# VIS4ROB-lab/ccm_slam

Measured on AMD Instinct MI355X. Metric: global-BA LM iterations/s (4-agent merged map), higher is better.
Workload: dtype f64; 1 GPU; gba_c4: global BA (MapFusionGBA numerics), 2000 KFs / 150000 landmarks / 954782 observations, Huber sqrt(5.99), landmark-sharded x1

## Files before the change

ccm_slam_amd/csrc/ba.hip:

```cpp
#include "common.h"
#include "test_internal.h"
#include "ba_types.h"
#include "lane_xor.h"
#include "ba_math.h"
#include <algorithm>
#include <chrono>
#include <cmath>
#include <cstring>
#include <limits>
#include <numeric>

int ccm_allreduce_f64(ccm_ctx* ctx, double* d_buf, size_t n);
int ccm_allreduce_max_f64(ccm_ctx* ctx, double* d_buf, size_t n);

namespace {


inline double now_ms() {
  return std::chrono::duration<double, std::milli>(std::chrono::steady_clock::now().time_since_epoch()).count();
}

__device__ __forceinline__ double wave_sum(double v) { return lanex::wave_sum(v); }

__device__ __forceinline__ double block_sum(double v, double* lds ) {
// ... 2634 lines not shown
    if (d.chunk_off) hipLaunchKernelGGL(ba_backsub_chi2_e, dim3(d.n_chunk), dim3(kTPB), 0, ctx->stream, d, ba->cur, 0.0, 1);
    else hipLaunchKernelGGL(ba_backsub_chi2, dim3(d.n_wg_pt), dim3(kTPB), 0, ctx->stream, d, ba->cur, 0.0, 1);
  }
  hipMemsetAsync(d.part_cam, 0, sizeof(double) * d.n_wg_cam, ctx->stream);
  const bool poll = ba->nranks == 1 && poll_enabled();
  const unsigned long long ticket = ++ba->rb_ticket;
  hipLaunchKernelGGL(ba_reduce_scalars, dim3(1), dim3(kTPB), 0, ctx->stream, d, ba->stop_local(), 0, 0, poll ? ba->h_rb : (double*)nullptr, ticket);
  RC(ba_allreduce_sum(ba, d.scal, 4));
  double s[6];
  if (poll) { RC(read_scalars_polled(ba, s, nullptr, ticket)); } else { RC(read_scalars(ba, s)); }
  *chi = s[0];
  ba->stop_any = s[2] > 0.0;
  return CCM_OK;
}

int build_system(ccm_ba* ba, double lambda_next = -1.0) {
  ccm_ctx* ctx = ba->ctx;
  BaDev& d = ba->d;
  ba->dinv_done_lambda = -1.0;
  if (d.Lloc) {
    ccm_prof_scope ps(ctx, CCM_K_BA_LINEARIZE);
    if (d.chunk_off) {
      hipLaunchKernelGGL(ba_linearize_pts_e, dim3(d.n_chunk), dim3(kTPB), 0, ctx->stream, d, ba->cur, lambda_next);
      if (lambda_next >= 0.0) ba->dinv_done_lambda = lambda_next;
    } else hipLaunchKernelGGL(ba_linearize_pts, dim3(d.n_wg_pt), dim3(kTPB), 0, ctx->stream, d, ba->cur);
  }
  if (d.Cp) {
    ccm_prof_scope ps(ctx, CCM_K_BA_CAM);
    hipLaunchKernelGGL(ba_linearize_cams, dim3(d.n_wg_wave4), dim3(kTPB), 0, ctx->stream, d, ba->cur);
  }
  CCM_HIP_CHECK(ctx, hipGetLastError());
  return CCM_OK;
}

int max_diag(ccm_ba* ba, double* out) {
  ccm_ctx* ctx = ba->ctx;
  BaDev& d = ba->d;
  const double* hpp = d.Hpp;
  if (ba->nranks > 1 && d.Cp) {
    CCM_HIP_CHECK(ctx, hipMemcpyAsync(ba->d_hpp_full, d.Hpp, 36 * (size_t)d.Cp * sizeof(double), hipMemcpyDeviceToDevice, ctx->stream));
    RC(ba_allreduce_sum(ba, ba->d_hpp_full, 36 * (size_t)d.Cp));
    hpp = ba->d_hpp_full;
  }
  const int nb = std::max(1, std::min(d.n_wg_pt, 512));
  hipLaunchKernelGGL(ba_maxdiag, dim3(nb), dim3(kTPB), 0, ctx->stream, d, hpp, d.part_pt, nb, 0);
  hipLaunchKernelGGL(ba_maxdiag, dim3(1), dim3(kTPB), 0, ctx->stream, d, hpp, d.part_pt, nb, 1);
  RC(ba_allreduce_max(ba, d.scal + 4, 1));
  double s[6];
  RC(read_scalars(ba, s));
  *out = s[4];
  return CCM_OK;
}

__global__ void ba_f64_to_f32(const double* __restrict__ in, float* __restrict__ out, size_t n) {
  const size_t i = (size_t)blockIdx.x * blockDim.x + threadIdx.x;
  if (i < n) out[i] = (float)in[i];
}

int coarse_build(ccm_ba* ba, double lambda) {
  ccm_ctx* ctx = ba->ctx;
  BaDev& d = ba->d;
  ccm_prof_scope ps(ctx, CCM_K_BA_COARSE);
  const int Nc = ba->coarse_Nc, na = ba->coarse_na, nn = na + 1;
  hipLaunchKernelGGL(ba_coarse_P, dim3(ccm_div_up(d.Cp, kTPB)), dim3(kTPB), 0, ctx->stream, d, ba->cur, ba->d_cP);
  hipLaunchKernelGGL(ba_coarse_assemble, dim3(ba->coarse_ncb), dim3(kCoarseTPB), 0, ctx->stream, d, (const double*)ba->d_cP,
                     (const int*)ba->d_cb_off, (const int*)ba->d_cb_ent, ba->coarse_ncb, (const int*)ba->d_blk_i, (const int*)ba->d_blk_j, lambda, ba->d_cstage);
  hipLaunchKernelGGL(ba_coarse_sum, dim3(ccm_div_up((int64_t)Nc * Nc, kTPB)), dim3(kTPB), 0, ctx->stream, (const double*)ba->d_cstage, (const unsigned*)ba->d_cb_key,
                     ba->coarse_ncb, na, nn, ba->d_cA, Nc);
  CCM_HIP_CHECK(ctx, hipGetLastError());
  RC(ccm_dense_chol_inverse_dev(ctx, ba->d_cA, Nc, ba->d_cLinv, ba->d_cX, ba->d_cAinv, ba->d_cinfo));
  if (ba->d_cAinv32) {
    const size_t n = (size_t)Nc * Nc;
    hipLaunchKernelGGL(ba_f64_to_f32, dim3((unsigned)ccm_div_up((int64_t)n, kTPB)), dim3(kTPB), 0, ctx->stream, (const double*)ba->d_cAinv, ba->d_cAinv32, n);
    CCM_HIP_CHECK(ctx, hipGetLastError());
  }
  return CCM_OK;
}

int coarse_prepare(ccm_ba* ba, double lambda) {
  const double win = 16.0;
  const double win_up_env = 0.0;
  const double win_up = win_up_env > 0 ? win_up_env : (ba->pers_grid ? 64.0 : win);
  const bool need = !ba->coarse_reuse || !ba->coarse_valid || ba->coarse_stale_bad || lambda > win_up * ba->coarse_lambda_built || lambda < ba->coarse_lambda_built / win;
  ba->coarse_fresh = need;
  if (!need) return CCM_OK;
  RC(coarse_build(ba, lambda));
  ba->coarse_valid = true; ba->coarse_stale_bad = false; ba->coarse_lambda_built = lambda;
  return CCM_OK;
}

int lm_trial(ccm_ba* ba, double lambda, const ccm_ba_options& opt, double* temp_chi, double* scale, bool* ok, int* pcg_iters) {
  ccm_ctx* ctx = ba->ctx;
  BaDev& d = ba->d;
  const int cur = ba->cur;
  if (!ba->pers_grid && ba->pers_grid_built && ba->pers_cooldown > 0 && --ba->pers_cooldown == 0) ba->pers_grid = ba->pers_grid_built;
  if (d.Lloc && ba->dinv_done_lambda != lambda) {
    ccm_prof_scope ps(ctx, CCM_K_BA_DINV);
    hipLaunchKernelGGL(ba_dinv, dim3(d.n_wg_pt), dim3(kTPB), 0, ctx->stream, d, lambda);
  }
  ba->dinv_done_lambda = -1.0;
  *ok = true;
  *pcg_iters = 0;
  bool small_path = false, pers_trial = false, pers_launch_failed = false, cams_updated = false;
  int small_flags[4] = {0, 0, 0, 0};
  if (d.Cp) {
    RC(launch_schur(ba));
    RC(ba_allreduce_sum(ba, ba->d_red, ba->red_count));
    const double tol_default = 1e-8;
    const double tol = opt.pcg_rel_tol > 0 ? opt.pcg_rel_tol : tol_default;
    const int max_it = opt.pcg_max_iters > 0 ? opt.pcg_max_iters : 1000;
    int flags[4] = {0, 0, 0, 0};
    const bool dense2_on = true;
    if (ba->d_cholreg_L) {
      CCM_LDS_ATTR(ctx, CCM_LDS_BA_CHOLREG, ba_solve_cholreg, cholreg_lds_bytes());
      if (!ba->cholreg_table_built) {
        hipLaunchKernelGGL(ba_cholreg_table, dim3(1), dim3(kCRTPB), 0, ctx->stream, d, ba->d_cholreg_tab);
        ba->cholreg_table_built = true;
      }
      {
        ccm_prof_scope ps(ctx, CCM_K_BA_PCG_PERSIST);
        hipLaunchKernelGGL(ba_solve_cholreg, dim3(1), dim3(kCRTPB), cholreg_lds_bytes(), ctx->stream, d, lambda, ba->d_cholreg_L, (const int*)ba->d_cholreg_tab,
                           ccm_dbg("cholreg") ? (long long*)ba->d_cholreg_dbg : (long long*)nullptr, cur, ba->rank == 0 ? 1 : 0);
      }
      small_path = true;
      cams_updated = true;
    } else if (d.Cp > kSmallMaxCp && d.Cp <= kDense2MaxCp && ba->d_dense_T && ba->d_pers_coff && dense2_on) {
      CCM_LDS_ATTR(ctx, CCM_LDS_BA_DENSE2, ba_solve_dense2, dense2_lds_bytes());
      {
// ... 537 lines not shown
```

ccm_slam_amd/csrc/common.h:

```cpp
#pragma once
#include <hip/hip_runtime.h>
#if defined(__HIP_DEVICE_COMPILE__) && !defined(__gfx950__)
#error "libccm_hip.so is written for gfx950 (MI355X) only: build with --offload-arch=gfx950"
#endif
#include <stdint.h>
#include <map>
#include <cstring>
#include <string>
#include <vector>
#include <mutex>
#include "../../include/ccm_hip.h"

struct ccm_prof_slot {
  std::vector<std::pair<hipEvent_t, hipEvent_t>> pending;
  int64_t launches = 0;
  double total_ms = 0.0;
};

struct ccm_ctx {
  int device = 0;
  hipStream_t stream = nullptr;
  std::string err;
  int prof_class = -2;
  ccm_prof_slot prof[CCM_K_COUNT];
// ... 12 lines not shown
int ccm_set_error(ccm_ctx* ctx, int code, const std::string& msg);
bool ccm_dbg(const char* topic);

struct ccm_coresident_scope {
  ccm_ctx* ctx; bool chained = false;
  explicit ccm_coresident_scope(ccm_ctx* c);
  ~ccm_coresident_scope();
  ccm_coresident_scope(const ccm_coresident_scope&) = delete;
  ccm_coresident_scope& operator=(const ccm_coresident_scope&) = delete;
};
void ccm_coresident_note_abort(ccm_ctx* ctx);

#define CCM_HIP_CHECK(ctx, expr)                                                        \
  do {                                                                                  \
    hipError_t _e = (expr);                                                             \
    if (_e != hipSuccess)                                                               \
      return ccm_set_error((ctx), CCM_E_HIP,                                            \
                           std::string(#expr) + ": " + hipGetErrorString(_e) + " (" +   \
                               __FILE__ + ":" + std::to_string(__LINE__) + ")");        \
  } while (0)

enum { CCM_LDS_BA_ROW = 0, CCM_LDS_BA_ROW2 = 8, CCM_LDS_BA_SMALL, CCM_LDS_BA_TILES, CCM_LDS_PG_PRECOND, CCM_LDS_POSEOPT, CCM_LDS_SIM3OPT, CCM_LDS_BA_DENSE2, CCM_LDS_ORB_OCT, CCM_LDS_ORB_OCT2, CCM_LDS_BA_ROW3, CCM_LDS_BA_ROW4, CCM_LDS_POSEOPT1, CCM_LDS_BA_CHOLREG };
#define CCM_LDS_ATTR(ctx, bit, func, bytes)                                                                              \
  do {                                                                                                                   \
    if (!((ctx)->lds_attr_done & (1u << (bit)))) {                                                                       \
      CCM_HIP_CHECK((ctx), hipFuncSetAttribute((const void*)(func), hipFuncAttributeMaxDynamicSharedMemorySize, (int)(bytes))); \
      (ctx)->lds_attr_done |= 1u << (bit);                                                                               \
    }                                                                                                                    \
  } while (0)

struct ccm_prof_scope {
  ccm_ctx* ctx; int cls; hipStream_t st = nullptr; hipEvent_t e0 = nullptr, e1 = nullptr; bool on = false;
  ccm_prof_scope(ccm_ctx* c, int k, hipStream_t launch_stream = nullptr);
  ~ccm_prof_scope();
};

int ccm_scratch(ccm_ctx* ctx, size_t bytes, void** out);
int ccm_io_scratch(ccm_ctx* ctx, size_t bytes, void** out);
int ccm_pin_scratch(ccm_ctx* ctx, size_t bytes, void** out);
int ccm_pool_get(ccm_ctx* ctx, size_t bytes, void** out, size_t* actual);
void ccm_pool_put(ccm_ctx* ctx, void* p, size_t actual);
struct ccm_tile_plan {
  int T = 0;
  std::vector<int> h_col_off;
  std::vector<int> h_upd_off;
  std::vector<int> h_row_off;
  const int* d_col_rows = nullptr;
  const int* d_upd_pairs = nullptr;
  const int* d_row_cols = nullptr;
};
void ccm_tile_plan_symbolic(int T, const std::vector<char>& nz, ccm_tile_plan* plan, std::vector<int>* col_rows, std::vector<int>* upd_pairs,
                            std::vector<int>* row_cols);
int ccm_dense_chol_solve_dev(ccm_ctx* ctx, double* d_A, int N, double* d_b, double* d_linv, int* d_info, const ccm_tile_plan* plan = nullptr);
int ccm_dense_chol_inverse_dev(ccm_ctx* ctx, double* d_A, int N, double* d_linv, double* d_X, double* d_Ainv, int* d_info);
struct ccm_tsc {
  int T = 0, n_tiles = 0, n_levels = 0;
  std::vector<int> tid;
  std::vector<int> lvl_col_off, lvl_gt_off, lvl_pt_off;
  int *d_tid = nullptr, *d_cols = nullptr, *d_gt = nullptr, *d_gk_off = nullptr, *d_gk = nullptr, *d_pt = nullptr;
  int *d_rc_off = nullptr, *d_rc = nullptr, *d_cr_off = nullptr, *d_cr = nullptr;
  double *d_tiles = nullptr, *d_linv = nullptr;
  int* d_info = nullptr;
  std::vector<std::pair<void*, size_t>> blocks;
  ccm_ctx* owner = nullptr;
  ccm_tsc() = default;
  ccm_tsc(const ccm_tsc&) = delete;
  ccm_tsc& operator=(const ccm_tsc&) = delete;
  ~ccm_tsc();
};
int ccm_tsc_create(ccm_ctx* ctx, int T, const std::vector<char>& nz, ccm_tsc* out);
void ccm_tsc_destroy(ccm_ctx* ctx, ccm_tsc* p);
int ccm_tsc_clear(ccm_ctx* ctx, ccm_tsc* p);
int ccm_tsc_solve(ccm_ctx* ctx, ccm_tsc* p, double* d_b);
static inline size_t ccm_align256(size_t n) { return (n + 255) & ~(size_t)255; }

static inline int ccm_div_up(int64_t a, int64_t b) { return (int)((a + b - 1) / b); }
```

ccm_slam_amd/csrc/dense_chol.hip:

```cpp
#include "common.h"
#include "test_internal.h"
#include <cstdlib>
#include <cstring>
#include <vector>

namespace {

constexpr int NB = 64;
constexpr int LD = NB + 1;
constexpr int kTPB = 256;
typedef double v4d __attribute__((ext_vector_type(4)));

__device__ __forceinline__ void tile_abt(const double* As, const double* Bs, v4d acc[4], int wave, int lane) {
  const int i = lane & 15, kq = lane >> 4;
#pragma unroll 4
  for (int kk = 0; kk < NB / 4; kk++) {
    const int k = 4 * kk + kq;
    const double a = As[(16 * wave + i) * LD + k];
#pragma unroll
    for (int s = 0; s < 4; s++) {
      const double b = Bs[(16 * s + i) * LD + k];
      acc[s] = __builtin_amdgcn_mfma_f64_16x16x4f64(a, b, acc[s], 0, 0, 0);
    }
  }
}

__device__ __forceinline__ void load_tile(double* dst, const double* src, int ld_src) {
  double v[NB * NB / kTPB];
#pragma unroll
  for (int q = 0; q < NB * NB / kTPB; q++) { const int e = threadIdx.x + q * kTPB; v[q] = src[(size_t)(e / NB) * ld_src + e % NB]; }
#pragma unroll
  for (int q = 0; q < NB * NB / kTPB; q++) { const int e = threadIdx.x + q * kTPB; dst[(e / NB) * LD + e % NB] = v[q]; }
}

__device__ __forceinline__ double bcast64(double v, int lane) {
  const long long b = __double_as_longlong(v);
  const int lo = __builtin_amdgcn_readlane((int)(b & 0xffffffffll), lane), hi = __builtin_amdgcn_readlane((int)(b >> 32), lane);
  return __longlong_as_double(((long long)hi << 32) | (unsigned int)lo);
}
__device__ __forceinline__ void chol_diag_body(double* Ajj, size_t N, int j, double* Lg, int* info) {
  constexpr int LR = NB + 2;
  __shared__ __attribute__((aligned(16))) double L[NB * LR];
  __shared__ double rdiag[NB];
  const int lane = threadIdx.x & 63;
  const int wv = __builtin_amdgcn_readfirstlane(threadIdx.x >> 6);
  {
    double tmp[NB / 2];
#pragma unroll
    for (int r = 0; r < NB / 2; r++) tmp[r] = Ajj[(size_t)(wv * (NB / 2) + r) * N + lane];
#pragma unroll
    for (int r = 0; r < NB / 2; r++) L[(wv * (NB / 2) + r) * LR + lane] = tmp[r];
  }
  __syncthreads();
  int bad_col = 0;
  double row[NB], cur[NB], nxt[NB];
  double x[NB];
  if (wv == 0) {
#pragma unroll
    for (int k = 0; k < NB; k++) { row[k] = L[lane * LR + k]; cur[k] = 0.0; nxt[k] = 0.0; }
  }
  __syncthreads();
#pragma unroll
  for (int c = 0; c <= NB; c++) {
    if (wv == 0) {
      if (c < NB) {
        double acc[4] = {row[c], 0.0, 0.0, 0.0};
#pragma unroll
        for (int k = 0; k < c; k++) acc[k & 3] = __builtin_fma(-row[k], cur[k], acc[k & 3]);
        if (c + 1 < NB) {
#pragma unroll
          for (int k = 0; k < c; k++) nxt[k] = L[(c + 1) * LR + k];
        }
        const double sv = (acc[0] + acc[1]) + (acc[2] + acc[3]);
        double dd = bcast64(sv, c);
        if (!(dd > 0.0)) { if (!bad_col) bad_col = c + 1; dd = 1.0; }
        const double inv = rsqrt(dd), l = dd * inv;
        row[c] = (lane == c) ? l : sv * inv;
        L[lane * LR + c] = row[c];
        if (lane == c) rdiag[c] = inv;
        if (c + 1 < NB) nxt[c] = bcast64(row[c], c + 1);
#pragma unroll
        for (int k = 0; k <= c; k++) cur[k] = nxt[k];
      }
    } else if (c >= 1) {
      const int r = c - 1;
      const double* Lrow = L + r * LR;
      double acc[4] = {(r == lane) ? 1.0 : 0.0, 0.0, 0.0, 0.0};
#pragma unroll
      for (int k = 0; k < r; k++) acc[k & 3] = __builtin_fma(-Lrow[k], x[k], acc[k & 3]);
      x[r] = ((acc[0] + acc[1]) + (acc[2] + acc[3])) * rdiag[r];
      Lg[r * NB + lane] = x[r];
    }
    __syncthreads();
  }
  if (wv == 0) {
    if (bad_col && lane == 0 && *info == 0) *info = j * NB + bad_col;
#pragma unroll
    for (int r = 0; r < NB; r++) Ajj[(size_t)r * N + lane] = (lane <= r) ? L[r * LR + lane] : 0.0;
  }
}
__device__ __forceinline__ void chol_diag_body_blk(double* Ajj, size_t N, int j, double* Lg, int* info) {
  constexpr int LR = NB + 2, KB = 16;
  __shared__ __attribute__((aligned(16))) double L[NB * LR];
  __shared__ double rdiag[NB];
  const int lane = threadIdx.x & 63;
  const int wv = __builtin_amdgcn_readfirstlane(threadIdx.x >> 6);
  {
    double tmp[NB / 2];
#pragma unroll
    for (int r = 0; r < NB / 2; r++) tmp[r] = Ajj[(size_t)(wv * (NB / 2) + r) * N + lane];
#pragma unroll
    for (int r = 0; r < NB / 2; r++) L[(wv * (NB / 2) + r) * LR + lane] = tmp[r];
  }
  __syncthreads();
  constexpr int kBlocks = NB / KB;
  static_assert(NB % KB == 0 && kBlocks >= 1, "both waves must run the same whole number of 16-column blocks");
  if (wv == 0) {
    int bad_col = 0;
#pragma unroll
    for (int b = 0; b < kBlocks; b++) {
      const int c0 = KB * b;
      double row[KB];
#pragma unroll
      for (int c = 0; c < KB; c += 2) { const double2 v = *reinterpret_cast<const double2*>(&L[lane * LR + c0 + c]); row[c] = v.x; row[c + 1] = v.y; }
#pragma unroll 2
      for (int k = 0; k < c0; k += 2) {
        const double2 a2 = *reinterpret_cast<const double2*>(&L[lane * LR + k]);
#pragma unroll
        for (int c = 0; c < KB; c++) {
          const double2 l2 = *reinterpret_cast<const double2*>(&L[(c0 + c) * LR + k]);
          row[c] = __builtin_fma(-a2.y, l2.y, __builtin_fma(-a2.x, l2.x, row[c]));
        }
      }
#pragma unroll
      for (int c = 0; c < KB; c++) {
        double s0 = row[c], s1 = 0.0;
#pragma unroll
        for (int k = 0; k < c; k++) {
          const double m = bcast64(row[k], c0 + c);
          if (k & 1) s1 = __builtin_fma(-row[k], m, s1); else s0 = __builtin_fma(-row[k], m, s0);
        }
        const double sv = s0 + s1;
        double dd = bcast64(sv, c0 + c);
        if (!(dd > 0.0)) { if (!bad_col) bad_col = c0 + c + 1; dd = 1.0; }
        const double inv = rsqrt(dd);
        row[c] = (lane == c0 + c) ? dd * inv : sv * inv;
        if (lane == c0 + c) rdiag[c0 + c] = inv;
      }
#pragma unroll
      for (int c = 0; c < KB; c += 2) { double2 v; v.x = row[c]; v.y = row[c + 1]; *reinterpret_cast<double2*>(&L[lane * LR + c0 + c]) = v; }
      __syncthreads();
    }
    if (bad_col && lane == 0 && *info == 0) *info = j * NB + bad_col;
#pragma unroll
    for (int r = 0; r < NB; r++) Ajj[(size_t)r * N + lane] = (lane <= r) ? L[r * LR + lane] : 0.0;
  } else {
    double x[NB];
#pragma unroll
    for (int b = 0; b < kBlocks; b++) {
      __syncthreads();
#pragma unroll
      for (int rr = 0; rr < KB; rr++) {
        const int r = KB * b + rr;
        const double* Lrow = L + r * LR;
        double acc[4] = {(r == lane) ? 1.0 : 0.0, 0.0, 0.0, 0.0};
#pragma unroll
        for (int k = 0; k < r; k++) acc[k & 3] = __builtin_fma(-Lrow[k], x[k], acc[k & 3]);
        x[r] = ((acc[0] + acc[1]) + (acc[2] + acc[3])) * rdiag[r];
        Lg[r * NB + lane] = x[r];
        asm volatile("" ::: "memory");
// ... 134 lines not shown
  __shared__ double v[NB];
  const int t = threadIdx.x;
  const double* Li = Linv_all + (size_t)j * NB * NB;
  v[t] = b[(size_t)j * NB + t];
  __syncthreads();
  double s = 0;
  if (!transpose) { for (int k = 0; k <= t; k++) s += Li[t * NB + k] * v[k]; }
  else { for (int k = t; k < NB; k++) s += Li[k * NB + t] * v[k]; }
  b[(size_t)j * NB + t] = s;
}
__global__ __launch_bounds__(NB) void chol_solve_update(const double* A, int N, double* b, int j, int transpose, const int* list ) {
  __shared__ double v[NB];
  const int t = threadIdx.x;
  v[t] = b[(size_t)j * NB + t];
  __syncthreads();
  double s = 0;
  if (!transpose) {
    const int i = list ? list[blockIdx.x] : j + 1 + blockIdx.x;
    const double* Lij = A + ((size_t)i * NB + t) * N + (size_t)j * NB;
    for (int k = 0; k < NB; k++) s += Lij[k] * v[k];
    b[(size_t)i * NB + t] -= s;
  } else {
    const int k = list ? list[blockIdx.x] : blockIdx.x;
    const double* Ljk = A + ((size_t)j * NB) * N + (size_t)k * NB + t;
    for (int r = 0; r < NB; r++) s += Ljk[(size_t)r * N] * v[r];
    b[(size_t)k * NB + t] -= s;
  }
}

__device__ __forceinline__ void load_tile_t(double* dst, const double* src, int ld_src) {
  double v[NB * NB / kTPB];
#pragma unroll
  for (int q = 0; q < NB * NB / kTPB; q++) { const int e = threadIdx.x + q * kTPB; v[q] = src[(size_t)(e / NB) * ld_src + e % NB]; }
#pragma unroll
  for (int q = 0; q < NB * NB / kTPB; q++) { const int e = threadIdx.x + q * kTPB; dst[(e % NB) * LD + e / NB] = v[q]; }
}

__device__ __forceinline__ void tile_abt16(const double* As, const double* Bs, v4d& acc, int wave, int lane) {
  const int i = lane & 15, kq = lane >> 4;
#pragma unroll 4
  for (int kk = 0; kk < NB / 4; kk++) {
    const int k = 4 * kk + kq;
    acc = __builtin_amdgcn_mfma_f64_16x16x4f64(As[(16 * wave + i) * LD + k], Bs[i * LD + k], acc, 0, 0, 0);
  }
}
__device__ __forceinline__ void load_strip_t(double* dst, const double* src, int ld_src) {
  double v[NB * 16 / kTPB];
#pragma unroll
  for (int q = 0; q < NB * 16 / kTPB; q++) { const int e = threadIdx.x + q * kTPB; v[q] = src[(size_t)(e / 16) * ld_src + e % 16]; }
#pragma unroll
  for (int q = 0; q < NB * 16 / kTPB; q++) { const int e = threadIdx.x + q * kTPB; dst[(e % 16) * LD + e / 16] = v[q]; }
}

__global__ __launch_bounds__(kTPB) void chol_tri_diag(int N, const double* Linv_all, double* X) {
  const int j = blockIdx.x;
  for (int e = threadIdx.x; e < NB * NB; e += kTPB) X[((size_t)j * NB + e / NB) * N + (size_t)j * NB + e % NB] = Linv_all[(size_t)j * NB * NB + e];
}
__global__ __launch_bounds__(kTPB) void chol_tri_step(const double* A, int N, const double* Linv_all, double* X, int k) {
  __shared__ double As[NB * LD], Bs[16 * LD];
  const int nj = k + 1;
  const int i = k + 1 + (int)blockIdx.x / nj, j = (int)blockIdx.x % nj, c0 = 16 * blockIdx.y;
  const int wave = threadIdx.x >> 6, lane = threadIdx.x & 63;
  const int i16 = lane & 15, kq = lane >> 4;
  double* Xij = X + ((size_t)i * NB) * N + (size_t)j * NB + c0;
  v4d acc = {0, 0, 0, 0};
  if (j != k) {
#pragma unroll
    for (int r = 0; r < 4; r++) acc[r] = Xij[(size_t)(16 * wave + kq + 4 * r) * N + i16];
  }
  load_tile(As, A + ((size_t)i * NB) * N + (size_t)k * NB, N);
  load_strip_t(Bs, X + ((size_t)k * NB) * N + (size_t)j * NB + c0, N);
  __syncthreads();
  tile_abt16(As, Bs, acc, wave, lane);
  __syncthreads();
  if (i == k + 1) {
#pragma unroll
    for (int r = 0; r < 4; r++) Bs[i16 * LD + 16 * wave + kq + 4 * r] = acc[r];
    load_tile(As, Linv_all + (size_t)i * NB * NB, NB);
    __syncthreads();
    v4d out = {0, 0, 0, 0};
    tile_abt16(As, Bs, out, wave, lane);
#pragma unroll
    for (int r = 0; r < 4; r++) Xij[(size_t)(16 * wave + kq + 4 * r) * N + i16] = -out[r];
  } else {
#pragma unroll
    for (int r = 0; r < 4; r++) Xij[(size_t)(16 * wave + kq + 4 * r) * N + i16] = acc[r];
  }
}

__global__ __launch_bounds__(kTPB) void chol_xtx(const double* X, int N, double* Ainv) {
  __shared__ double As[NB * LD], Bs[16 * LD];
  const int T = N / NB;
  const int pi = blockIdx.x, c0 = 16 * blockIdx.y;
  int p = (int)((sqrtf(8.0f * (float)pi + 1.0f) - 1.0f) * 0.5f);
  while (p * (p + 1) / 2 > pi) p--;
  while ((p + 1) * (p + 2) / 2 <= pi) p++;
  const int q = pi - p * (p + 1) / 2;
  const int wave = threadIdx.x >> 6, lane = threadIdx.x & 63;
  const int i16 = lane & 15, kq = lane >> 4;
  v4d acc = {0, 0, 0, 0};
  for (int k = p; k < T; k++) {
    load_tile_t(As, X + ((size_t)k * NB) * N + (size_t)p * NB, N);
    load_strip_t(Bs, X + ((size_t)k * NB) * N + (size_t)q * NB + c0, N);
    __syncthreads();
    tile_abt16(As, Bs, acc, wave, lane);
    __syncthreads();
  }
#pragma unroll
  for (int r = 0; r < 4; r++) {
    const int row = 16 * wave + kq + 4 * r, col = c0 + i16;
    Ainv[((size_t)p * NB + row) * N + (size_t)q * NB + col] = acc[r];
    if (p != q) Ainv[((size_t)q * NB + col) * N + (size_t)p * NB + row] = acc[r];
  }
}

}

int ccm_dense_chol_solve_dev(ccm_ctx* ctx, double* d_A, int N, double* d_b, double* d_linv, int* d_info, const ccm_tile_plan* plan) {
  if (N % NB) return ccm_set_error(ctx, CCM_E_ARG, "dense cholesky: N must be a multiple of 64");
  const int T = N / NB;
  if (plan && (plan->T != T || T >= 32768)) return ccm_set_error(ctx, CCM_E_ARG, "dense cholesky: tile plan does not match");
  CCM_HIP_CHECK(ctx, hipMemsetAsync(d_info, 0, sizeof(int), ctx->stream));
  for (int j = 0; j < T; j++) {
    if (diag_blocked()) hipLaunchKernelGGL(chol_diag_wave_blk, dim3(1), dim3(128), 0, ctx->stream, d_A, N, j, d_linv, d_info);
    else hipLaunchKernelGGL(chol_diag_wave, dim3(1), dim3(128), 0, ctx->stream, d_A, N, j, d_linv, d_info);
    if (plan) {
      const int nr = plan->h_col_off[j + 1] - plan->h_col_off[j], np = plan->h_upd_off[j + 1] - plan->h_upd_off[j];
      if (nr) hipLaunchKernelGGL(chol_panel, dim3(nr), dim3(kTPB), 0, ctx->stream, d_A, N, j, (const double*)d_linv, plan->d_col_rows + plan->h_col_off[j]);
      if (np) hipLaunchKernelGGL(chol_update, dim3(np), dim3(kTPB), 0, ctx->stream, d_A, N, j, plan->d_upd_pairs + plan->h_upd_off[j]);
      continue;
    }
    const int rem = T - j - 1;
    if (rem > 0) {
      hipLaunchKernelGGL(chol_panel, dim3(rem), dim3(kTPB), 0, ctx->stream, d_A, N, j, (const double*)d_linv, (const int*)nullptr);
      hipLaunchKernelGGL(chol_update, dim3(rem * (rem + 1) / 2), dim3(kTPB), 0, ctx->stream, d_A, N, j, (const int*)nullptr);
    }
  }
  for (int j = 0; j < T; j++) {
    hipLaunchKernelGGL(chol_solve_diag, dim3(1), dim3(NB), 0, ctx->stream, d_b, j, (const double*)d_linv, 0);
    if (plan) {
      const int nr = plan->h_col_off[j + 1] - plan->h_col_off[j];
      if (nr) hipLaunchKernelGGL(chol_solve_update, dim3(nr), dim3(NB), 0, ctx->stream, (const double*)d_A, N, d_b, j, 0, plan->d_col_rows + plan->h_col_off[j]);
    } else if (T - j - 1 > 0) hipLaunchKernelGGL(chol_solve_update, dim3(T - j - 1), dim3(NB), 0, ctx->stream, (const double*)d_A, N, d_b, j, 0, (const int*)nullptr);
  }
  for (int j = T - 1; j >= 0; j--) {
    hipLaunchKernelGGL(chol_solve_diag, dim3(1), dim3(NB), 0, ctx->stream, d_b, j, (const double*)d_linv, 1);
    if (plan) {
      const int nc = plan->h_row_off[j + 1] - plan->h_row_off[j];
      if (nc) hipLaunchKernelGGL(chol_solve_update, dim3(nc), dim3(NB), 0, ctx->stream, (const double*)d_A, N, d_b, j, 1, plan->d_row_cols + plan->h_row_off[j]);
    } else if (j > 0) hipLaunchKernelGGL(chol_solve_update, dim3(j), dim3(NB), 0, ctx->stream, (const double*)d_A, N, d_b, j, 1, (const int*)nullptr);
  }
  CCM_HIP_CHECK(ctx, hipGetLastError());
  return CCM_OK;
}

void ccm_tile_plan_symbolic(int T, const std::vector<char>& nz_in, ccm_tile_plan* plan, std::vector<int>* col_rows, std::vector<int>* upd_pairs,
                            std::vector<int>* row_cols) {
  std::vector<char> nz = nz_in;
  plan->T = T;
  plan->h_col_off.assign(1, 0); plan->h_upd_off.assign(1, 0); plan->h_row_off.assign(1, 0);
  col_rows->clear(); upd_pairs->clear(); row_cols->clear();
  std::vector<int> rows;
  for (int j = 0; j < T; j++) {
    rows.clear();
    for (int i = j + 1; i < T; i++) if (nz[(size_t)i * T + j]) rows.push_back(i);
// ... 128 lines not shown
  CCM_HIP_CHECK(ctx, hipMalloc(&dA, Ap.size() * sizeof(double)));
  CCM_HIP_CHECK(ctx, hipMalloc(&db, N * sizeof(double)));
  CCM_HIP_CHECK(ctx, hipMalloc(&dl, (size_t)N * NB * sizeof(double)));
  CCM_HIP_CHECK(ctx, hipMalloc(&di, sizeof(int)));
  hipMemcpyAsync(dA, Ap.data(), Ap.size() * sizeof(double), hipMemcpyHostToDevice, ctx->stream);
  hipMemcpyAsync(db, bp.data(), N * sizeof(double), hipMemcpyHostToDevice, ctx->stream);
  int rc = ccm_dense_chol_solve_dev(ctx, dA, N, db, dl, di);
  if (rc == CCM_OK) {
    hipMemcpyAsync(bp.data(), db, N * sizeof(double), hipMemcpyDeviceToHost, ctx->stream);
    hipMemcpyAsync(info, di, sizeof(int), hipMemcpyDeviceToHost, ctx->stream);
    if (hipStreamSynchronize(ctx->stream) != hipSuccess) rc = ccm_set_error(ctx, CCM_E_HIP, "ccm_debug_dense_solve: sync");
    for (int i = 0; i < n; i++) x[i] = bp[i];
  }
  hipFree(dA); hipFree(db); hipFree(dl); hipFree(di);
  return rc;
}

int ccm_internal::debug_tile_solve(ccm_ctx* ctx, const double* A, const double* b, int n, double* x, int* info, int* levels, int* tiles) {
  if (!ctx || !A || !b || !x || !info || n <= 0) return ccm_set_error(ctx, CCM_E_ARG, "ccm_debug_tile_solve: bad args");
  CCM_HIP_CHECK(ctx, hipSetDevice(ctx->device));
  const int N = ((n + NB - 1) / NB) * NB, T = N / NB;
  std::vector<char> nz((size_t)T * T, 0);
  for (int i = 0; i < n; i++) for (int c = 0; c <= i; c++) if (A[(size_t)i * n + c] != 0.0) nz[(size_t)(i / NB) * T + c / NB] = 1;
  for (int t = 0; t < T; t++) nz[(size_t)t * T + t] = 1;
  ccm_tsc p;
  if (int rc = ccm_tsc_create(ctx, T, nz, &p)) return rc;
  std::vector<double> ht((size_t)p.n_tiles * NB * NB, 0.0), hb(N, 0.0);
  for (int i = 0; i < N; i++) {
    if (i >= n) { ht[(size_t)p.tid[(size_t)(i / NB) * T + i / NB] * NB * NB + (size_t)(i % NB) * (NB + 1)] = 1.0; continue; }
    hb[i] = b[i];
    for (int c = 0; c <= i; c++) {
      const double v = A[(size_t)i * n + c];
      if (v != 0.0) ht[(size_t)p.tid[(size_t)(i / NB) * T + c / NB] * NB * NB + (size_t)(i % NB) * NB + c % NB] = v;
    }
  }
  double* db = nullptr;
  CCM_HIP_CHECK(ctx, hipMalloc(&db, N * sizeof(double)));
  hipMemcpyAsync(p.d_tiles, ht.data(), ht.size() * sizeof(double), hipMemcpyHostToDevice, ctx->stream);
  hipMemcpyAsync(db, hb.data(), N * sizeof(double), hipMemcpyHostToDevice, ctx->stream);
  int rc = ccm_tsc_solve(ctx, &p, db);
  if (rc == CCM_OK) {
    hipMemcpyAsync(hb.data(), db, N * sizeof(double), hipMemcpyDeviceToHost, ctx->stream);
    hipMemcpyAsync(info, p.d_info, sizeof(int), hipMemcpyDeviceToHost, ctx->stream);
    if (hipStreamSynchronize(ctx->stream) != hipSuccess) rc = ccm_set_error(ctx, CCM_E_HIP, "ccm_debug_tile_solve: sync");
    for (int i = 0; i < n; i++) x[i] = hb[i];
  }
  if (levels) *levels = p.n_levels;
  if (tiles) *tiles = p.n_tiles;
  hipStreamSynchronize(ctx->stream);
  hipFree(db);
  return rc;
}

int ccm_dense_chol_inverse_dev(ccm_ctx* ctx, double* d_A, int N, double* d_linv, double* d_X, double* d_Ainv, int* d_info) {
  if (N % NB) return ccm_set_error(ctx, CCM_E_ARG, "dense cholesky: N must be a multiple of 64");
  const int T = N / NB;
  CCM_HIP_CHECK(ctx, hipMemsetAsync(d_info, 0, sizeof(int), ctx->stream));
  for (int j = 0; j < T; j++) {
    if (diag_blocked()) hipLaunchKernelGGL(chol_diag_wave_blk, dim3(1), dim3(128), 0, ctx->stream, d_A, N, j, d_linv, d_info);
    else hipLaunchKernelGGL(chol_diag_wave, dim3(1), dim3(128), 0, ctx->stream, d_A, N, j, d_linv, d_info);
    const int rem = T - j - 1;
    if (rem > 0) {
      hipLaunchKernelGGL(chol_panel, dim3(rem), dim3(kTPB), 0, ctx->stream, d_A, N, j, (const double*)d_linv, (const int*)nullptr);
      hipLaunchKernelGGL(chol_update, dim3(rem * (rem + 1) / 2), dim3(kTPB), 0, ctx->stream, d_A, N, j, (const int*)nullptr);
    }
  }
  hipLaunchKernelGGL(chol_tri_diag, dim3(T), dim3(kTPB), 0, ctx->stream, N, (const double*)d_linv, d_X);
  for (int k = 0; k + 1 < T; k++)
    hipLaunchKernelGGL(chol_tri_step, dim3((T - k - 1) * (k + 1), NB / 16), dim3(kTPB), 0, ctx->stream, (const double*)d_A, N, (const double*)d_linv, d_X, k);
  hipLaunchKernelGGL(chol_xtx, dim3(T * (T + 1) / 2, NB / 16), dim3(kTPB), 0, ctx->stream, (const double*)d_X, N, d_Ainv);
  CCM_HIP_CHECK(ctx, hipGetLastError());
  return CCM_OK;
}

int ccm_internal::debug_dense_inverse(ccm_ctx* ctx, const double* A, int n, double* Ainv, int* info) {
  if (!ctx || !A || !Ainv || !info || n <= 0) return ccm_set_error(ctx, CCM_E_ARG, "ccm_debug_dense_inverse: bad args");
  CCM_HIP_CHECK(ctx, hipSetDevice(ctx->device));
  const int N = ((n + NB - 1) / NB) * NB;
  std::vector<double> Ap((size_t)N * N, 0.0);
  for (int i = 0; i < N; i++) {
    if (i < n) { for (int c = 0; c < n; c++) Ap[(size_t)i * N + c] = A[(size_t)i * n + c]; }
    else Ap[(size_t)i * N + i] = 1.0;
  }
  double *dA = nullptr, *dl = nullptr, *dX = nullptr, *dI = nullptr; int* di = nullptr;
  CCM_HIP_CHECK(ctx, hipMalloc(&dA, Ap.size() * sizeof(double)));
  CCM_HIP_CHECK(ctx, hipMalloc(&dX, Ap.size() * sizeof(double)));
  CCM_HIP_CHECK(ctx, hipMalloc(&dI, Ap.size() * sizeof(double)));
  CCM_HIP_CHECK(ctx, hipMalloc(&dl, (size_t)N * NB * sizeof(double)));
  CCM_HIP_CHECK(ctx, hipMalloc(&di, sizeof(int)));
  hipMemcpyAsync(dA, Ap.data(), Ap.size() * sizeof(double), hipMemcpyHostToDevice, ctx->stream);
  hipMemsetAsync(dX, 0, Ap.size() * sizeof(double), ctx->stream);
  int rc = ccm_dense_chol_inverse_dev(ctx, dA, N, dl, dX, dI, di);
  if (rc == CCM_OK) {
    hipMemcpyAsync(Ap.data(), dI, Ap.size() * sizeof(double), hipMemcpyDeviceToHost, ctx->stream);
    hipMemcpyAsync(info, di, sizeof(int), hipMemcpyDeviceToHost, ctx->stream);
    if (hipStreamSynchronize(ctx->stream) != hipSuccess) rc = ccm_set_error(ctx, CCM_E_HIP, "ccm_debug_dense_inverse: sync");
    for (int i = 0; i < n; i++) for (int c = 0; c < n; c++) Ainv[(size_t)i * n + c] = Ap[(size_t)i * N + c];
  }
  hipFree(dA); hipFree(dX); hipFree(dI); hipFree(dl); hipFree(di);
  return rc;
}
```

Baseline: 928.6 LM iter/s.

## Fuse dense Cholesky inverse stages to cut kernel launches in coarse preconditioner

Restructures the dense Cholesky-based inverse of the coarse preconditioner matrix. Each factorization step now fuses the panel solve, trailing update and the next diagonal factorization into one kernel (chol_step), and the info memset moves into the first diagonal kernel. The per-column triangular inverse steps become a single kernel with double-buffered LDS prefetch (chol_tri_cols). The f64-to-f32 conversion is folded into chol_xtx. This removes many small launches and serialized passes. The cost is redundant recomputation of panel tiles across blocks, and the diagonal work now runs in a single block at the tail of each step.

```diff
diff --git a/ccm_slam_amd/csrc/ba.hip b/ccm_slam_amd/csrc/ba.hip
--- a/ccm_slam_amd/csrc/ba.hip
+++ b/ccm_slam_amd/csrc/ba.hip
@@ -2710,11 +2710,6 @@
   return CCM_OK;
 }
 
-__global__ void ba_f64_to_f32(const double* __restrict__ in, float* __restrict__ out, size_t n) {
-  const size_t i = (size_t)blockIdx.x * blockDim.x + threadIdx.x;
-  if (i < n) out[i] = (float)in[i];
-}
-
 int coarse_build(ccm_ba* ba, double lambda) {
   ccm_ctx* ctx = ba->ctx;
   BaDev& d = ba->d;
@@ -2726,12 +2721,7 @@
   hipLaunchKernelGGL(ba_coarse_sum, dim3(ccm_div_up((int64_t)Nc * Nc, kTPB)), dim3(kTPB), 0, ctx->stream, (const double*)ba->d_cstage, (const unsigned*)ba->d_cb_key,
                      ba->coarse_ncb, na, nn, ba->d_cA, Nc);
   CCM_HIP_CHECK(ctx, hipGetLastError());
-  RC(ccm_dense_chol_inverse_dev(ctx, ba->d_cA, Nc, ba->d_cLinv, ba->d_cX, ba->d_cAinv, ba->d_cinfo));
-  if (ba->d_cAinv32) {
-    const size_t n = (size_t)Nc * Nc;
-    hipLaunchKernelGGL(ba_f64_to_f32, dim3((unsigned)ccm_div_up((int64_t)n, kTPB)), dim3(kTPB), 0, ctx->stream, (const double*)ba->d_cAinv, ba->d_cAinv32, n);
-    CCM_HIP_CHECK(ctx, hipGetLastError());
-  }
+  RC(ccm_dense_chol_inverse_dev(ctx, ba->d_cA, Nc, ba->d_cLinv, ba->d_cX, ba->d_cAinv, ba->d_cinfo, ba->d_cAinv32));
   return CCM_OK;
 }
 
diff --git a/ccm_slam_amd/csrc/common.h b/ccm_slam_amd/csrc/common.h
--- a/ccm_slam_amd/csrc/common.h
+++ b/ccm_slam_amd/csrc/common.h
@@ -88,7 +88,7 @@
 void ccm_tile_plan_symbolic(int T, const std::vector<char>& nz, ccm_tile_plan* plan, std::vector<int>* col_rows, std::vector<int>* upd_pairs,
                             std::vector<int>* row_cols);
 int ccm_dense_chol_solve_dev(ccm_ctx* ctx, double* d_A, int N, double* d_b, double* d_linv, int* d_info, const ccm_tile_plan* plan = nullptr);
-int ccm_dense_chol_inverse_dev(ccm_ctx* ctx, double* d_A, int N, double* d_linv, double* d_X, double* d_Ainv, int* d_info);
+int ccm_dense_chol_inverse_dev(ccm_ctx* ctx, double* d_A, int N, double* d_linv, double* d_X, double* d_Ainv, int* d_info, float* d_Ainv32 );
 struct ccm_tsc {
   int T = 0, n_tiles = 0, n_levels = 0;
   std::vector<int> tid;
diff --git a/ccm_slam_amd/csrc/dense_chol.hip b/ccm_slam_amd/csrc/dense_chol.hip
--- a/ccm_slam_amd/csrc/dense_chol.hip
+++ b/ccm_slam_amd/csrc/dense_chol.hip
@@ -44,7 +44,7 @@
   __shared__ double rdiag[NB];
   const int lane = threadIdx.x & 63;
   const int wv = __builtin_amdgcn_readfirstlane(threadIdx.x >> 6);
-  {
+  if (wv < 2) {
     double tmp[NB / 2];
 #pragma unroll
     for (int r = 0; r < NB / 2; r++) tmp[r] = Ajj[(size_t)(wv * (NB / 2) + r) * N + lane];
@@ -82,7 +82,7 @@
 #pragma unroll
         for (int k = 0; k <= c; k++) cur[k] = nxt[k];
       }
-    } else if (c >= 1) {
+    } else if (wv == 1 && c >= 1) {
       const int r = c - 1;
       const double* Lrow = L + r * LR;
       double acc[4] = {(r == lane) ? 1.0 : 0.0, 0.0, 0.0, 0.0};
@@ -105,7 +105,7 @@
   __shared__ double rdiag[NB];
   const int lane = threadIdx.x & 63;
   const int wv = __builtin_amdgcn_readfirstlane(threadIdx.x >> 6);
-  {
+  if (wv < 2) {
     double tmp[NB / 2];
 #pragma unroll
     for (int r = 0; r < NB / 2; r++) tmp[r] = Ajj[(size_t)(wv * (NB / 2) + r) * N + lane];
@@ -115,7 +115,10 @@
   __syncthreads();
   constexpr int kBlocks = NB / KB;
   static_assert(NB % KB == 0 && kBlocks >= 1, "both waves must run the same whole number of 16-column blocks");
-  if (wv == 0) {
+  if (wv >= 2) {
+#pragma unroll
+    for (int b = 0; b < kBlocks; b++) __syncthreads();
+  } else if (wv == 0) {
     int bad_col = 0;
 #pragma unroll
     for (int b = 0; b < kBlocks; b++) {
@@ -356,43 +359,133 @@
   for (int q = 0; q < NB * 16 / kTPB; q++) { const int e = threadIdx.x + q * kTPB; dst[(e % 16) * LD + e / 16] = v[q]; }
 }
 
-__global__ __launch_bounds__(kTPB) void chol_tri_diag(int N, const double* Linv_all, double* X) {
-  const int j = blockIdx.x;
-  for (int e = threadIdx.x; e < NB * NB; e += kTPB) X[((size_t)j * NB + e / NB) * N + (size_t)j * NB + e % NB] = Linv_all[(size_t)j * NB * NB + e];
-}
-__global__ __launch_bounds__(kTPB) void chol_tri_step(const double* A, int N, const double* Linv_all, double* X, int k) {
-  __shared__ double As[NB * LD], Bs[16 * LD];
-  const int nj = k + 1;
-  const int i = k + 1 + (int)blockIdx.x / nj, j = (int)blockIdx.x % nj, c0 = 16 * blockIdx.y;
+template <bool kBlocked>
+__global__ __launch_bounds__(128) void chol_diag_first(double* A, int N, double* Linv_all, int* info) {
+  if (threadIdx.x == 0) *info = 0;
+  if (kBlocked) chol_diag_body_blk(A, (size_t)N, 0, Linv_all, info);
+  else chol_diag_body(A, (size_t)N, 0, Linv_all, info);
+}
+__device__ __forceinline__ void store_acc_lds(double* dst, const v4d acc[4], int wave, int lane) {
+#pragma unroll
+  for (int s = 0; s < 4; s++)
+#pragma unroll
+    for (int r = 0; r < 4; r++) dst[(16 * wave + (lane >> 4) + 4 * r) * LD + 16 * s + (lane & 15)] = acc[s][r];
+}
+template <bool kBlocked>
+__global__ __launch_bounds__(kTPB) void chol_step(double* A, int N, int j, double* Linv_all, int* info) {
+  __shared__ double As[NB * LD], Bs[NB * LD], Cs[NB * LD];
+  const int rem = N / NB - j - 1;
+  int p = blockIdx.x, kk = 0;
+  while (p >= rem - kk) { p -= rem - kk; kk++; }
+  const int i = j + 1 + kk + p, k = j + 1 + kk;
+  const int wave = threadIdx.x >> 6, lane = threadIdx.x & 63;
+  {
+    constexpr int Q = NB * NB / kTPB;
+    const double* a = A + ((size_t)i * NB) * N + (size_t)j * NB;
+    const double* b = Linv_all + (size_t)j * NB * NB;
+    const double* c = A + ((size_t)k * NB) * N + (size_t)j * NB;
+    double va[Q], vb[Q], vc[Q];
+#pragma unroll
+    for (int q = 0; q < Q; q++) { const int e = threadIdx.x + q * kTPB; va[q] = a[(size_t)(e / NB) * N + e % NB]; vb[q] = b[e]; }
+    if (i != k) {
+#pragma unroll
+      for (int q = 0; q < Q; q++) { const int e = threadIdx.x + q * kTPB; vc[q] = c[(size_t)(e / NB) * N + e % NB]; }
+    }
+#pragma unroll
+    for (int q = 0; q < Q; q++) { const int e = threadIdx.x + q * kTPB; As[(e / NB) * LD + e % NB] = va[q]; Bs[(e / NB) * LD + e % NB] = vb[q]; }
+    if (i != k) {
+#pragma unroll
+      for (int q = 0; q < Q; q++) { const int e = threadIdx.x + q * kTPB; Cs[(e / NB) * LD + e % NB] = vc[q]; }
+    }
+  }
+  __syncthreads();
+  v4d li[4] = {{0, 0, 0, 0}, {0, 0, 0, 0}, {0, 0, 0, 0}, {0, 0, 0, 0}}, lk[4] = {{0, 0, 0, 0}, {0, 0, 0, 0}, {0, 0, 0, 0}, {0, 0, 0, 0}};
+  tile_abt(As, Bs, li, wave, lane);
+  if (i != k) tile_abt(Cs, Bs, lk, wave, lane);
+  __syncthreads();
+  store_acc_lds(As, li, wave, lane);
+  if (i != k) store_acc_lds(Cs, lk, wave, lane);
+  else {
+    double* Lij = A + ((size_t)j * NB) * N + (size_t)i * NB;
+#pragma unroll
+    for (int s = 0; s < 4; s++)
+#pragma unroll
+      for (int r = 0; r < 4; r++) Lij[(size_t)(16 * wave + (lane >> 4) + 4 * r) * N + 16 * s + (lane & 15)] = li[s][r];
+  }
+  __syncthreads();
+  v4d acc[4] = {{0, 0, 0, 0}, {0, 0, 0, 0}, {0, 0, 0, 0}, {0, 0, 0, 0}};
+  tile_abt(As, i != k ? Cs : As, acc, wave, lane);
+  double* Aik = A + ((size_t)i * NB) * N + (size_t)k * NB;
+#pragma unroll
+  for (int s = 0; s < 4; s++)
+#pragma unroll
+    for (int r = 0; r < 4; r++) Aik[(size_t)(16 * wave + (lane >> 4) + 4 * r) * N + 16 * s + (lane & 15)] -= acc[s][r];
+  if (blockIdx.x != 0) return;
+  __syncthreads();
+  if (kBlocked) chol_diag_body_blk(Aik, (size_t)N, j + 1, Linv_all + (size_t)(j + 1) * NB * NB, info);
+  else chol_diag_body(Aik, (size_t)N, j + 1, Linv_all + (size_t)(j + 1) * NB * NB, info);
+}
+
+__global__ __launch_bounds__(kTPB) void chol_tri_cols(const double* A, int N, const double* Linv_all, double* X) {
+  __shared__ double As[2][NB * LD], Bs[2][16 * LD];
+  const int T = N / NB, j = blockIdx.x, c0 = 16 * blockIdx.y;
   const int wave = threadIdx.x >> 6, lane = threadIdx.x & 63;
   const int i16 = lane & 15, kq = lane >> 4;
-  double* Xij = X + ((size_t)i * NB) * N + (size_t)j * NB + c0;
+  constexpr int QA = NB * NB / kTPB, QB = NB * 16 / kTPB;
+  const double* Lij = Linv_all + (size_t)j * NB * NB + c0;
+  for (int e = threadIdx.x; e < NB * 16; e += kTPB) X[((size_t)j * NB + e / 16) * N + (size_t)j * NB + c0 + e % 16] = Lij[(size_t)(e / 16) * NB + e % 16];
+  if (j + 1 >= T) return;
+  double va[QA], vb[QB];
+  auto fetch = [&](int i, int k) {
+    const double* a = (k < i) ? A + ((size_t)k * NB) * N + (size_t)i * NB : Linv_all + (size_t)i * NB * NB;
+    const int lda = (k < i) ? N : NB;
+#pragma unroll
+    for (int q = 0; q < QA; q++) { const int e = threadIdx.x + q * kTPB; va[q] = a[(size_t)(e / NB) * lda + e % NB]; }
+    if (k < i) {
+      const double* b = (k == j) ? Lij : X + ((size_t)k * NB) * N + (size_t)j * NB + c0;
+      const int ldb = (k == j) ? NB : N;
+#pragma unroll
+      for (int q = 0; q < QB; q++) { const int e = threadIdx.x + q * kTPB; vb[q] = b[(size_t)(e / 16) * ldb + e % 16]; }
+    }
+  };
+  auto commit = [&](int buf, bool with_b) {
+#pragma unroll
+    for (int q = 0; q < QA; q++) { const int e = threadIdx.x + q * kTPB; As[buf][(e / NB) * LD + e % NB] = va[q]; }
+    if (with_b) {
+#pragma unroll
+      for (int q = 0; q < QB; q++) { const int e = threadIdx.x + q * kTPB; Bs[buf][(e % 16) * LD + e / 16] = vb[q]; }
+    }
+  };
+  int i = j + 1, k = j, buf = 0;
+  fetch(i, k);
+  commit(0, true);
   v4d acc = {0, 0, 0, 0};
-  if (j != k) {
-#pragma unroll
-    for (int r = 0; r < 4; r++) acc[r] = Xij[(size_t)(16 * wave + kq + 4 * r) * N + i16];
-  }
-  load_tile(As, A + ((size_t)i * NB) * N + (size_t)k * NB, N);
-  load_strip_t(Bs, X + ((size_t)k * NB) * N + (size_t)j * NB + c0, N);
-  __syncthreads();
-  tile_abt16(As, Bs, acc, wave, lane);
-  __syncthreads();
-  if (i == k + 1) {
-#pragma unroll
-    for (int r = 0; r < 4; r++) Bs[i16 * LD + 16 * wave + kq + 4 * r] = acc[r];
-    load_tile(As, Linv_all + (size_t)i * NB * NB, NB);
+  while (i < T) {
     __syncthreads();
-    v4d out = {0, 0, 0, 0};
-    tile_abt16(As, Bs, out, wave, lane);
-#pragma unroll
-    for (int r = 0; r < 4; r++) Xij[(size_t)(16 * wave + kq + 4 * r) * N + i16] = -out[r];
-  } else {
-#pragma unroll
-    for (int r = 0; r < 4; r++) Xij[(size_t)(16 * wave + kq + 4 * r) * N + i16] = acc[r];
-  }
-}
-
-__global__ __launch_bounds__(kTPB) void chol_xtx(const double* X, int N, double* Ainv) {
+    int ni = i, nk = k + 1;
+    if (k == i) { ni = i + 1; nk = j; }
+    const bool more = ni < T;
+    if (more) fetch(ni, nk);
+    if (k < i) {
+      tile_abt16(As[buf], Bs[buf], acc, wave, lane);
+      if (k == i - 1) {
+#pragma unroll
+        for (int r = 0; r < 4; r++) Bs[buf ^ 1][i16 * LD + 16 * wave + kq + 4 * r] = acc[r];
+      }
+    } else {
+      v4d out = {0, 0, 0, 0};
+      tile_abt16(As[buf], Bs[buf], out, wave, lane);
+      double* Xij = X + ((size_t)i * NB) * N + (size_t)j * NB + c0;
+#pragma unroll
+      for (int r = 0; r < 4; r++) Xij[(size_t)(16 * wave + kq + 4 * r) * N + i16] = -out[r];
+      acc = v4d{0, 0, 0, 0};
+    }
+    if (more) commit(buf ^ 1, nk < ni);
+    buf ^= 1; i = ni; k = nk;
+  }
+}
+
+__global__ __launch_bounds__(kTPB) void chol_xtx(const double* X, int N, double* Ainv, float* Ainv32 ) {
   __shared__ double As[NB * LD], Bs[16 * LD];
   const int T = N / NB;
   const int pi = blockIdx.x, c0 = 16 * blockIdx.y;
@@ -415,6 +508,10 @@
     const int row = 16 * wave + kq + 4 * r, col = c0 + i16;
     Ainv[((size_t)p * NB + row) * N + (size_t)q * NB + col] = acc[r];
     if (p != q) Ainv[((size_t)q * NB + col) * N + (size_t)p * NB + row] = acc[r];
+    if (Ainv32) {
+      Ainv32[((size_t)p * NB + row) * N + (size_t)q * NB + col] = (float)acc[r];
+      if (p != q) Ainv32[((size_t)q * NB + col) * N + (size_t)p * NB + row] = (float)acc[r];
+    }
   }
 }
 
@@ -649,23 +746,18 @@
   return rc;
 }
 
-int ccm_dense_chol_inverse_dev(ccm_ctx* ctx, double* d_A, int N, double* d_linv, double* d_X, double* d_Ainv, int* d_info) {
+int ccm_dense_chol_inverse_dev(ccm_ctx* ctx, double* d_A, int N, double* d_linv, double* d_X, double* d_Ainv, int* d_info, float* d_Ainv32) {
   if (N % NB) return ccm_set_error(ctx, CCM_E_ARG, "dense cholesky: N must be a multiple of 64");
   const int T = N / NB;
-  CCM_HIP_CHECK(ctx, hipMemsetAsync(d_info, 0, sizeof(int), ctx->stream));
-  for (int j = 0; j < T; j++) {
-    if (diag_blocked()) hipLaunchKernelGGL(chol_diag_wave_blk, dim3(1), dim3(128), 0, ctx->stream, d_A, N, j, d_linv, d_info);
-    else hipLaunchKernelGGL(chol_diag_wave, dim3(1), dim3(128), 0, ctx->stream, d_A, N, j, d_linv, d_info);
+  if (diag_blocked()) hipLaunchKernelGGL(chol_diag_first<true>, dim3(1), dim3(128), 0, ctx->stream, d_A, N, d_linv, d_info);
+  else hipLaunchKernelGGL(chol_diag_first<false>, dim3(1), dim3(128), 0, ctx->stream, d_A, N, d_linv, d_info);
+  for (int j = 0; j + 1 < T; j++) {
     const int rem = T - j - 1;
-    if (rem > 0) {
-      hipLaunchKernelGGL(chol_panel, dim3(rem), dim3(kTPB), 0, ctx->stream, d_A, N, j, (const double*)d_linv, (const int*)nullptr);
-      hipLaunchKernelGGL(chol_update, dim3(rem * (rem + 1) / 2), dim3(kTPB), 0, ctx->stream, d_A, N, j, (const int*)nullptr);
-    }
-  }
-  hipLaunchKernelGGL(chol_tri_diag, dim3(T), dim3(kTPB), 0, ctx->stream, N, (const double*)d_linv, d_X);
-  for (int k = 0; k + 1 < T; k++)
-    hipLaunchKernelGGL(chol_tri_step, dim3((T - k - 1) * (k + 1), NB / 16), dim3(kTPB), 0, ctx->stream, (const double*)d_A, N, (const double*)d_linv, d_X, k);
-  hipLaunchKernelGGL(chol_xtx, dim3(T * (T + 1) / 2, NB / 16), dim3(kTPB), 0, ctx->stream, (const double*)d_X, N, d_Ainv);
+    if (diag_blocked()) hipLaunchKernelGGL(chol_step<true>, dim3(rem * (rem + 1) / 2), dim3(kTPB), 0, ctx->stream, d_A, N, j, d_linv, d_info);
+    else hipLaunchKernelGGL(chol_step<false>, dim3(rem * (rem + 1) / 2), dim3(kTPB), 0, ctx->stream, d_A, N, j, d_linv, d_info);
+  }
+  hipLaunchKernelGGL(chol_tri_cols, dim3(T, NB / 16), dim3(kTPB), 0, ctx->stream, (const double*)d_A, N, (const double*)d_linv, d_X);
+  hipLaunchKernelGGL(chol_xtx, dim3(T * (T + 1) / 2, NB / 16), dim3(kTPB), 0, ctx->stream, (const double*)d_X, N, d_Ainv, d_Ainv32);
   CCM_HIP_CHECK(ctx, hipGetLastError());
   return CCM_OK;
 }
@@ -687,7 +779,7 @@
   CCM_HIP_CHECK(ctx, hipMalloc(&di, sizeof(int)));
   hipMemcpyAsync(dA, Ap.data(), Ap.size() * sizeof(double), hipMemcpyHostToDevice, ctx->stream);
   hipMemsetAsync(dX, 0, Ap.size() * sizeof(double), ctx->stream);
-  int rc = ccm_dense_chol_inverse_dev(ctx, dA, N, dl, dX, dI, di);
+  int rc = ccm_dense_chol_inverse_dev(ctx, dA, N, dl, dX, dI, di, nullptr);
   if (rc == CCM_OK) {
     hipMemcpyAsync(Ap.data(), dI, Ap.size() * sizeof(double), hipMemcpyDeviceToHost, ctx->stream);
     hipMemcpyAsync(info, di, sizeof(int), hipMemcpyDeviceToHost, ctx->stream);
```

Result: slower. 916.0 LM iter/s (-1.4%).
